# sudhirverma/distributed-ranges

Measured on AMD Instinct MI355X. Metric: elements/s & % HBM roofline: reduce/scan/sort/SpMV at 1/2/4/8 MI355X, higher is better.
Workload: dtype f32

## Files before the change

distributed-ranges_amd/include/dr/shp/merge_sort.hpp:

```cpp
#pragma once

#include <hip/hip_runtime.h>

#include <algorithm>
#include <cstddef>
#include <cstdint>

namespace shp::detail::msort {

constexpr int kMsBlock = 256;
template <typename T> constexpr int ipt() {
  return sizeof(T) <= 4 ? 8 : sizeof(T) <= 8 ? 8 : sizeof(T) <= 16 ? 4 : sizeof(T) <= 32 ? 2 : 1;
}
template <typename T> constexpr int pad_every() { return ipt<T>() >= 4 ? ipt<T>() : 0; }
template <typename T> constexpr std::size_t padded(std::size_t e) {
  return pad_every<T>() ? e + e / pad_every<T>() : e;
}
#ifndef DR_SHP_MSORT_SORT_THREADS
#define DR_SHP_MSORT_SORT_THREADS 256
#endif
static_assert(DR_SHP_MSORT_SORT_THREADS >= kMsBlock && (DR_SHP_MSORT_SORT_THREADS & (DR_SHP_MSORT_SORT_THREADS - 1)) == 0,
              "DR_SHP_MSORT_SORT_THREADS must be a power of two and at least kMsBlock");
template <typename T> constexpr int sort_threads() {
  return padded<T>(std::size_t(DR_SHP_MSORT_SORT_THREADS) * ipt<T>()) * sizeof(T) <= 65536 ? DR_SHP_MSORT_SORT_THREADS
                                                                                         : kMsBlock;
}
template <typename T> constexpr std::size_t tile() { return std::size_t(kMsBlock) * ipt<T>(); }
template <typename T> constexpr std::size_t sort_tile() { return std::size_t(sort_threads<T>()) * ipt<T>(); }

template <typename I, typename PA, typename PB, typename Comp>
__host__ __device__ inline I merge_path(PA a, I na, PB b, I nb, I diag, Comp &comp) {
  I lo = diag > nb ? diag - nb : 0, hi = diag < na ? diag : na;
  while (lo < hi) {
    const I mid = (lo + hi) / 2;
    if (!comp(b[diag - 1 - mid], a[mid])) lo = mid + 1;
    else hi = mid;
  }
  return lo;
}

template <typename T> struct lds_view {
  T *s;
  int off;
  __device__ T &operator[](int i) const {
    const int j = off + i;
    return s[pad_every<T>() ? j + j / pad_every<T>() : j];
  }
  __device__ lds_view at(int o) const { return {s, off + o}; }
};

template <int N, typename T, typename Comp>
__device__ inline int serial_merge(lds_view<T> v, int ai, int aend, int bi, int bend, T (&y)[N], Comp &comp) {
  int cnt = 0;
#pragma unroll
  for (int k = 0; k < N; k++) {
    if (ai < aend || bi < bend) {
      const bool take_b = bi < bend && (ai >= aend || comp(v[bi], v[ai]));
      if (take_b) y[k] = v[bi++];
      else y[k] = v[ai++];
      cnt = k + 1;
    }
  }
  return cnt;
}

template <typename T, std::size_t E> struct lds_tile {
  alignas(alignof(T) > 16 ? alignof(T) : 16) unsigned char raw[padded<T>(E) * sizeof(T)];
  __device__ lds_view<T> view() { return {reinterpret_cast<T *>(raw), 0}; }
};

template <typename T, typename Comp>
__global__ __launch_bounds__(sort_threads<T>()) void block_sort_kernel(T *data, std::size_t n, Comp comp) {
  constexpr int NT = sort_threads<T>();
  constexpr int N = ipt<T>();
  constexpr int TILE = (int)sort_tile<T>();
  __shared__ lds_tile<T, sort_tile<T>()> lds;
  const lds_view<T> s = lds.view();
  const std::size_t base = (std::size_t)blockIdx.x * TILE;
  const int cnt = (int)std::min<std::size_t>(TILE, n - base);
  {
    T r[N];
#pragma unroll
    for (int k = 0; k < N; k++)
      if (k * NT + (int)threadIdx.x < cnt) r[k] = data[base + k * NT + threadIdx.x];
#pragma unroll
    for (int k = 0; k < N; k++)
      if (k * NT + (int)threadIdx.x < cnt) s[k * NT + threadIdx.x] = r[k];
  }
  __syncthreads();
  const int my = threadIdx.x * N;
  const int valid = std::max(0, std::min(N, cnt - my));
  T x[N];
#pragma unroll
  for (int k = 0; k < N; k++)
    if (k < valid) x[k] = s[my + k];
#pragma unroll
  for (int r = 0; r < N; r++) {
#pragma unroll
    for (int k = r & 1; k + 1 < N; k += 2)
      if (k + 1 < valid && comp(x[k + 1], x[k])) {
        const T t = x[k];
        x[k] = x[k + 1];
        x[k + 1] = t;
      }
  }
  __syncthreads();
#pragma unroll
  for (int k = 0; k < N; k++)
    if (k < valid) s[my + k] = x[k];
  __syncthreads();
  for (int coop = 2; coop <= NT; coop *= 2) {
    const int lane = threadIdx.x % coop;
    const int g0 = (threadIdx.x / coop) * coop * N, half = coop / 2 * N;
    const int a0 = std::min(g0, cnt), a1 = std::min(g0 + half, cnt), b1 = std::min(g0 + 2 * half, cnt);
    const int na = a1 - a0, nb = b1 - a1;
    const int diag = std::min(lane * N, na + nb);
    const int i = merge_path<int>(s.at(a0), na, s.at(a1), nb, diag, comp);
    T y[N];
    const int got = serial_merge<N>(s, a0 + i, a1, a1 + diag - i, b1, y, comp);
    __syncthreads();
#pragma unroll
    for (int k = 0; k < N; k++)
      if (k < got) s[a0 + diag + k] = y[k];
    __syncthreads();
  }
#pragma unroll
  for (int k = 0; k < N; k++)
    if (k * NT + (int)threadIdx.x < cnt) data[base + k * NT + threadIdx.x] = s[k * NT + threadIdx.x];
}

struct pass_geom {
  std::size_t n, w;
  bool single;
  __host__ __device__ std::size_t pair_base(std::size_t d) const { return single ? 0 : d / (2 * w) * (2 * w); }
  __host__ __device__ std::size_t pair_end(std::size_t pb) const { return single ? n : std::min(n, pb + 2 * w); }
  __host__ __device__ std::size_t na(std::size_t pb) const { return std::min(w, n - pb); }
};

template <typename T, typename Comp>
__global__ void merge_partition_kernel(const T *src, pass_geom g, std::size_t ntiles, std::size_t *part, Comp comp) {
  const std::size_t t = (std::size_t)blockIdx.x * blockDim.x + threadIdx.x;
  if (t >= ntiles) return;
  const std::size_t d = t * tile<T>();
  const std::size_t pb = g.pair_base(d), na = g.na(pb), nb = g.pair_end(pb) - pb - na;
  part[t] = merge_path<std::size_t>(src + pb, na, src + pb + na, nb, d - pb, comp);
}

template <typename T, typename Comp>
__global__ __launch_bounds__(kMsBlock) void merge_kernel(const T *src, T *dst, pass_geom g, std::size_t ntiles,
                                                         const std::size_t *part, Comp comp) {
  constexpr int N = ipt<T>();
  constexpr std::size_t TILE = tile<T>();
  __shared__ lds_tile<T, tile<T>()> lds;
  const lds_view<T> s = lds.view();
  const std::size_t t = blockIdx.x;
  const std::size_t d0 = t * TILE, pb = g.pair_base(d0), pe = g.pair_end(pb);
  const std::size_t d1 = std::min(d0 + TILE, pe);
  const std::size_t na = g.na(pb);
  const std::size_t i0 = part[t];
  const std::size_t i1 = (t + 1 < ntiles && (t + 1) * TILE < pe) ? part[t + 1] : na;
  const std::size_t j0 = (d0 - pb) - i0, j1 = (d1 - pb) - i1;
  const T *A = src + pb, *B = src + pb + na;
  const int la = (int)(i1 - i0), lb = (int)(j1 - j0);
  {
    T r[N];
#pragma unroll
    for (int k = 0; k < N; k++) {
      const int e = k * kMsBlock + threadIdx.x;
      if (e < la) r[k] = A[i0 + e];
      else if (e < la + lb) r[k] = B[j0 + (e - la)];
    }
#pragma unroll
    for (int k = 0; k < N; k++) {
      const int e = k * kMsBlock + threadIdx.x;
      if (e < la + lb) s[e] = r[k];
    }
  }
  __syncthreads();
  const int diag = std::min((int)threadIdx.x * N, la + lb);
  const int i = merge_path<int>(s, la, s.at(la), lb, diag, comp);
  T y[N];
  const int got = serial_merge<N>(s, i, la, la + diag - i, la + lb, y, comp);
  __syncthreads();
#pragma unroll
  for (int k = 0; k < N; k++)
    if (k < got) s[diag + k] = y[k];
  __syncthreads();
#pragma unroll
  for (int k = 0; k < N; k++)
    if (k * kMsBlock + (int)threadIdx.x < la + lb) dst[d0 + k * kMsBlock + threadIdx.x] = s[k * kMsBlock + threadIdx.x];
}

template <typename T> __global__ void gather_samples_kernel(const T *data, std::size_t stride, std::size_t ns, T *s) {
  const std::size_t j = (std::size_t)blockIdx.x * blockDim.x + threadIdx.x;
  if (j < ns) s[j] = data[j * stride];
}

template <typename T> constexpr std::size_t scratch_bytes(std::size_t n) {
  const std::size_t tiles = (n + tile<T>() - 1) / tile<T>();
  return ((n * sizeof(T) + 255) & ~std::size_t(255)) + (tiles + 1) * sizeof(std::size_t);
}

inline unsigned blocks_of(std::size_t n, std::size_t per) { return (unsigned)std::max<std::size_t>(1, (n + per - 1) / per); }

template <typename T, typename Comp>
void merge_pass(const T *src, T *dst, pass_geom g, std::size_t *part, Comp comp, hipStream_t st) {
  const std::size_t ntiles = (g.n + tile<T>() - 1) / tile<T>();
  hipLaunchKernelGGL((merge_partition_kernel<T, Comp>), dim3(blocks_of(ntiles, 256)), dim3(256), 0, st, src, g,
                     ntiles, part, comp);
  hipLaunchKernelGGL((merge_kernel<T, Comp>), dim3((unsigned)ntiles), dim3(kMsBlock), 0, st, src, dst, g, ntiles,
                     part, comp);
}

template <typename T, typename Comp>
void local_sort(T *data, std::size_t n, void *scratch, Comp comp, hipStream_t st) {
  if (n <= 1) return;
  T *tmp = static_cast<T *>(scratch);
  auto *part = reinterpret_cast<std::size_t *>(static_cast<char *>(scratch) + ((n * sizeof(T) + 255) & ~std::size_t(255)));
  hipLaunchKernelGGL((block_sort_kernel<T, Comp>), dim3(blocks_of(n, sort_tile<T>())), dim3(sort_threads<T>()), 0,
                     st, data, n, comp);
  T *src = data, *dst = tmp;
  for (std::size_t w = sort_tile<T>(); w < n; w *= 2) {
    merge_pass<T>(src, dst, pass_geom{n, w, false}, part, comp, st);
    std::swap(src, dst);
  }
  if (src != data) (void)hipMemcpyAsync(data, src, n * sizeof(T), hipMemcpyDeviceToDevice, st);
}

}
```

Before: 532.3 billion.

## Pick block-sort output buffer by pass parity; use nontemporal vectorized tile I/O

Counts the merge passes up front so the block-sort kernel writes into whichever buffer makes the final merge pass land in the original array. This removes the trailing device-to-device copy. Tile loads and stores in the block-sort and merge kernels now use nontemporal builtins, with 16-byte vector stores for full, aligned 4- and 8-byte-element tiles, to cut cache pollution and the number of store instructions. Nontemporal hints could hurt if the next pass would have hit in the cache.

```diff
diff --git a/distributed-ranges_amd/include/dr/shp/merge_sort.hpp b/distributed-ranges_amd/include/dr/shp/merge_sort.hpp
--- a/distributed-ranges_amd/include/dr/shp/merge_sort.hpp
+++ b/distributed-ranges_amd/include/dr/shp/merge_sort.hpp
@@ -5,6 +5,7 @@
 #include <algorithm>
 #include <cstddef>
 #include <cstdint>
+#include <type_traits>
 
 namespace shp::detail::msort {
 
@@ -69,8 +70,43 @@
   __device__ lds_view<T> view() { return {reinterpret_cast<T *>(raw), 0}; }
 };
 
-template <typename T, typename Comp>
-__global__ __launch_bounds__(sort_threads<T>()) void block_sort_kernel(T *data, std::size_t n, Comp comp) {
+typedef unsigned int ms_u32x4 __attribute__((ext_vector_type(4)));
+
+template <typename T> __device__ inline T load_once(const T *p) {
+  if constexpr (std::is_arithmetic<T>::value) return __builtin_nontemporal_load(p);
+  else return *p;
+}
+
+template <int NT, std::size_t TILE, typename T> __device__ inline void store_tile(lds_view<T> s, T *dst, int cnt) {
+  if constexpr (sizeof(T) == 4 || sizeof(T) == 8) {
+    if (cnt == (int)TILE && reinterpret_cast<std::uintptr_t>(dst) % 16 == 0) {
+      constexpr int PER = 16 / sizeof(T), NV = (int)(TILE / PER);
+      static_assert(TILE % PER == 0 && NV % NT == 0, "whole 16-byte vectors, the same number for every thread");
+#pragma unroll
+      for (int q = 0; q < NV / NT; q++) {
+        const int v = q * NT + (int)threadIdx.x;
+        T x[PER];
+#pragma unroll
+        for (int e = 0; e < PER; e++) x[e] = s[v * PER + e];
+        ms_u32x4 w;
+        __builtin_memcpy(&w, x, 16);
+        __builtin_nontemporal_store(w, reinterpret_cast<ms_u32x4 *>(dst) + v);
+      }
+      return;
+    }
+  }
+#pragma unroll
+  for (int k = 0; k < (int)(TILE / NT); k++) {
+    const int e = k * NT + (int)threadIdx.x;
+    if (e < cnt) {
+      if constexpr (std::is_arithmetic<T>::value) __builtin_nontemporal_store(s[e], dst + e);
+      else dst[e] = s[e];
+    }
+  }
+}
+
+template <typename T, typename Comp>
+__global__ __launch_bounds__(sort_threads<T>()) void block_sort_kernel(const T *src, T *dst, std::size_t n, Comp comp) {
   constexpr int NT = sort_threads<T>();
   constexpr int N = ipt<T>();
   constexpr int TILE = (int)sort_tile<T>();
@@ -82,7 +118,7 @@
     T r[N];
 #pragma unroll
     for (int k = 0; k < N; k++)
-      if (k * NT + (int)threadIdx.x < cnt) r[k] = data[base + k * NT + threadIdx.x];
+      if (k * NT + (int)threadIdx.x < cnt) r[k] = load_once(src + base + k * NT + threadIdx.x);
 #pragma unroll
     for (int k = 0; k < N; k++)
       if (k * NT + (int)threadIdx.x < cnt) s[k * NT + threadIdx.x] = r[k];
@@ -124,9 +160,7 @@
       if (k < got) s[a0 + diag + k] = y[k];
     __syncthreads();
   }
-#pragma unroll
-  for (int k = 0; k < N; k++)
-    if (k * NT + (int)threadIdx.x < cnt) data[base + k * NT + threadIdx.x] = s[k * NT + threadIdx.x];
+  store_tile<NT, sort_tile<T>()>(s, dst + base, cnt);
 }
 
 struct pass_geom {
@@ -167,8 +201,8 @@
 #pragma unroll
     for (int k = 0; k < N; k++) {
       const int e = k * kMsBlock + threadIdx.x;
-      if (e < la) r[k] = A[i0 + e];
-      else if (e < la + lb) r[k] = B[j0 + (e - la)];
+      if (e < la) r[k] = load_once(A + i0 + e);
+      else if (e < la + lb) r[k] = load_once(B + j0 + (e - la));
     }
 #pragma unroll
     for (int k = 0; k < N; k++) {
@@ -186,9 +220,7 @@
   for (int k = 0; k < N; k++)
     if (k < got) s[diag + k] = y[k];
   __syncthreads();
-#pragma unroll
-  for (int k = 0; k < N; k++)
-    if (k * kMsBlock + (int)threadIdx.x < la + lb) dst[d0 + k * kMsBlock + threadIdx.x] = s[k * kMsBlock + threadIdx.x];
+  store_tile<kMsBlock, tile<T>()>(s, dst + d0, la + lb);
 }
 
 template <typename T> __global__ void gather_samples_kernel(const T *data, std::size_t stride, std::size_t ns, T *s) {
@@ -217,14 +249,15 @@
   if (n <= 1) return;
   T *tmp = static_cast<T *>(scratch);
   auto *part = reinterpret_cast<std::size_t *>(static_cast<char *>(scratch) + ((n * sizeof(T) + 255) & ~std::size_t(255)));
+  int passes = 0;
+  for (std::size_t w = sort_tile<T>(); w < n; w *= 2) passes++;
+  T *src = passes % 2 ? tmp : data, *dst = passes % 2 ? data : tmp;
   hipLaunchKernelGGL((block_sort_kernel<T, Comp>), dim3(blocks_of(n, sort_tile<T>())), dim3(sort_threads<T>()), 0,
-                     st, data, n, comp);
-  T *src = data, *dst = tmp;
+                     st, static_cast<const T *>(data), src, n, comp);
   for (std::size_t w = sort_tile<T>(); w < n; w *= 2) {
     merge_pass<T>(src, dst, pass_geom{n, w, false}, part, comp, st);
     std::swap(src, dst);
   }
-  if (src != data) (void)hipMemcpyAsync(data, src, n * sizeof(T), hipMemcpyDeviceToDevice, st);
-}
-
-}
+}
+
+}
```

Measured after the change: 532.9 billion (median of 3 runs). No clear change (+0.1%).
